# William-gregory/SeaIceExtentForecasting

Measured on AMD Instinct MI355X. Metric: GP fits/sec (n x n fp64, kernel+Cholesky+predict), higher is better.
Workload: dtype f64; 1 GPU; configs[2]: n=8192 d=8 fp64 RBF GPR, 40 retrospective years x hyper-parameter grid, one step = fits_per_step fits in lockstep; lockstep_group_asked=160, grid=smoke, parallelism=years sharded over 1 GPU(s), no data-path collective

## Files before the change

### include/sigp_debug.h

```cpp
#ifndef SIGP_DEBUG_H
#define SIGP_DEBUG_H
#include "sigp.h"
#ifdef __cplusplus
extern "C" {
#endif
int sigp_debug_diag_stamps(sigp_handle* h, const double* A128, double* out_us, int nout);
int sigp_debug_time_diag(sigp_handle* h, const double* A128, int skip, int reps, double* ms_avg, double* L_out, double* Linv_out);
int sigp_debug_time_kbuild(sigp_handle* h, int n, int d, int nb, int kernel_id, int flags, int reps, double* ms_avg);
int sigp_debug_mfma_peak(sigp_handle* h, int blocks, int iters, double* tflops, double seed);
int sigp_debug_time_syrk(sigp_handle* h, int rt, int K, int patch, int small, int reps, double* ms_avg, double* tflops, int dbg,
                         double* clock_ghz);
int sigp_debug_stream_concurrency(sigp_handle* h, int nstreams, int reps, int blocks, int iters, int use_slot_streams, double* ms_out);
int sigp_debug_cumask_probe(sigp_handle* h, const unsigned* mask8, int blocks, unsigned* out2);

int sigp_debug_run_gemm(sigp_handle* h, int dtype, int cfg, const void* A, int64_t lda, const void* B, int64_t ldb, void* C, int64_t ldc, int K, int r0, int r1,
                        int c0, int c1, int lower, int ktri, int batch, int64_t sA, int64_t sB, int64_t sC, int zcount, int64_t zA, int64_t zB, int64_t zC,
                        int zshift, int ride_bi1, int ride_rows, int64_t a_elems, int64_t b_elems, int64_t c_elems);
int sigp_debug_run_strip(sigp_handle* h, int dtype, void* M, int64_t ld, const void* Mt, int64_t ldm, int rb0, int nstrips, int J, int Wp, int members, int64_t sM,
                         int64_t sMt, int64_t m_elems, int64_t mt_elems);
int sigp_debug_run_link(sigp_handle* h, int dtype, void* M, int64_t ld, int c, const void* Linv, void* scratch, int rows_ride, int members, int64_t sM, int64_t sL,
                        int64_t sS, int64_t m_elems, int64_t linv_elems, int64_t scratch_elems);
int sigp_debug_run_refined_solve(sigp_handle* h, int trans, void* A, int64_t lda, int rows, const void* W, int64_t ldw, const void* L, int64_t ldl, int members,
                                 int64_t sA, int64_t sW, int64_t sL, int64_t a_elems, int64_t w_elems, int64_t l_elems);

int sigp_debug_run_rowdot(sigp_handle* h, int dtype, const void* Mx, int64_t ld, int nrows, int K, int kmode, const void* Zin, int64_t ldzin, void* Zout, int64_t ldzout,
                          int nrhs, int sub, const void* Zadd, int pm_pw, int j_off, int members, int64_t sM, int64_t sZi, int64_t sZo, int64_t m_elems,
                          int64_t zin_elems, int64_t zout_elems);
int sigp_debug_run_coldot(sigp_handle* h, int dtype, const void* Mx, int64_t ld, int ncols, int K, const void* Zin, int64_t ldzin, void* Zout, int64_t ldzout, int nrhs,
                          int64_t m_elems, int64_t zin_elems, int64_t zout_elems);
int sigp_debug_f32_solve(sigp_handle* h, int which, double* rhs, int64_t n, int nrhs);
int sigp_debug_f32_get_inverse(sigp_handle* h, int which, float* out);
int sigp_debug_run_hindcast_adjoint(sigp_handle* h, int64_t lead, int64_t min_train, int sigma_mode, int criterion, double* out, int64_t ldo);
int sigp_debug_run_hindcast_w(sigp_handle* h, int which, const double* U, const double* Cb, const double* z, const double* zbar, double* W, int n, int n_pad,
                              int64_t ld, int lead, int members, int64_t sC, int64_t sZ, int64_t c_elems, int64_t z_elems);
// ... 15 lines not shown
```

### seaiceextentforecasting_amd/csrc/gemm_mfma.hpp

```cpp
#pragma once
#include <hip/hip_runtime.h>

namespace sigp {

typedef double d4 __attribute__((ext_vector_type(4)));
typedef double d2 __attribute__((ext_vector_type(2)));
typedef float f4 __attribute__((ext_vector_type(4)));
typedef float f2 __attribute__((ext_vector_type(2)));

template <typename T> struct Num;
template <> struct Num<double> {
  typedef d4 acc_t;  typedef d2 v16_t;  typedef d2 v2_t;
  static constexpr int NE = 2;
  static constexpr int KT = 16;
  static constexpr int LDP = 18;
  __device__ static inline acc_t mfma(double a, double b, acc_t c) { return __builtin_amdgcn_mfma_f64_16x16x4f64(a, b, c, 0, 0, 0); }
  __device__ static inline int drow(int lq, int r) { return lq + 4 * r; }
  __device__ static inline int cswz(int R) { return (R & 1) << 3; }
};
template <> struct Num<float> {
  typedef f4 acc_t;  typedef f4 v16_t;  typedef f2 v2_t;
  static constexpr int NE = 4;
  static constexpr int KT = 32;
  static constexpr int LDP = 36;
  __device__ static inline acc_t mfma(float a, float b, acc_t c) { return __builtin_amdgcn_mfma_f32_16x16x4f32(a, b, c, 0, 0, 0); }
  __device__ static inline int drow(int lq, int r) { return 4 * lq + r; }
  __device__ static inline int cswz(int R) { return ((R >> 2) & 3) << 2; }
};

constexpr int KT = Num<double>::KT;

// ... 279 lines not shown
```

### seaiceextentforecasting_amd/csrc/sigp.hip

```cpp
#include <hip/hip_runtime.h>

#include <algorithm>
#include <cmath>
#include <cstdarg>
#include <cstdio>
#include <cstring>
#include <functional>
#include <limits>
#ifdef SIGP_DEBUG_TOOLS
#include <map>
#endif
#include <mutex>
#include <thread>
#include <chrono>
#include <string>
#include <type_traits>
#include <vector>

#include "../../include/sigp.h"
#include <dlfcn.h>
#include <rccl/rccl.h>
#include "gemm_mfma.hpp"
#include "kernels_misc.hpp"
#include "potrf_diag.hpp"
// ... 169 lines not shown
  bool built = false, factored = false, fitted = false;
  double sigma_f = 0, nlml = 0;
  KParams kp{};
  bool outer_set = false;
  int opt_outer = 8;
  int opt_lookahead = 1;
  int opt_small_tiles = 320;
  int opt_tiny_tiles = 256;
  int opt_pan_priority = 1;
  int opt_panel_ll = 0;
  int opt_panel_mode = 2;
  int opt_strip_min = 512;
  int opt_diag_tiles = 1;
  int opt_ride_tiles = 1;
  int opt_accurate = 0;
  int opt_strip_tri = 1;
  int opt_update_dbg = 0;
  int opt_c_dma = 0;
  int ncu = 256;
  int opt_ride_reps = 0;
  int opt_kbuild_mfma = 2;
  int opt_diag_prio = 1;
  int opt_schedule = 0;
  int opt_trsm128 = 256;
  int opt_n64_tiles = 0;
  int opt_wide_tiles = 0;
  int opt_syrk_v2 = 1;
  int opt_patch = 0;
  int opt_xcd_chunks = 0;
  int opt_first_on_panel = 1;
// ... 189 lines not shown
template <typename T, int TM, int TN, int WM, int WN, int MODE, bool BT>
int launch_gemm_cfg(sigp_handle* h, hipStream_t st, const GemmArgsT<T>& g) {
  const int nt = gemm_grid_size(g.r0, g.r1, g.c0, g.c1, g.lower, g.patch);
  if (nt <= 0) return SIGP_OK;
  auto kern = gemm_mfma_kernel<T, TM, TN, WM, WN, MODE, BT>;
  constexpr int lds = gemm_lds_bytes<T, TM, TN, BT>();
  static AttrOnce attr;
  HIPCHK(h, attr.set(h->device, (const void*)kern, lds));
  hipLaunchKernelGGL(kern, dim3(nt, std::max(1, g.batch), std::max(1, g.zcount)), dim3(256), lds, st, g);
  HIPCHK(h, hipGetLastError());
  return SIGP_OK;
}
template <int TM, int TN, int WM, int WN, int MODE, bool BT>
int launch_gemm_cfg(sigp_handle* h, hipStream_t st, const GemmArgs& g) { return launch_gemm_cfg<double, TM, TN, WM, WN, MODE, BT>(h, st, g); }

template <typename T, bool SET>
int launch_syrk128_t(sigp_handle* h, hipStream_t st, const GemmArgsT<T>& g, bool may_persist = false) {
  const int nt = gemm_grid_size(g.r0, g.r1, g.c0, g.c1, g.lower, g.patch);
  if (nt <= 0) return SIGP_OK;
  if (!sy_row_stride_ok(g.lda, sizeof(T)) || !sy_row_stride_ok(g.ldb, sizeof(T))) return fail(h, SIGP_BAD_ARG, "syrk128: operand row stride beyond the tile's 32-bit DMA offsets");
  static AttrOnce attr;
  HIPCHK(h, attr.set(h->device, (const void*)syrk128_kernel<T, SET>, SY_LDS_BYTES));
#ifdef SIGP_DEBUG_TOOLS
  if (g.dbg & (3 | 512)) {
    auto go = [&](auto abl) -> int {
      constexpr int A = decltype(abl)::value;
      static AttrOnce attr_a;
      HIPCHK(h, attr_a.set(h->device, (const void*)syrk128_kernel<T, SET, false, A>, SY_LDS_BYTES));
      hipLaunchKernelGGL((syrk128_kernel<T, SET, false, A>), dim3(nt, std::max(1, g.batch), std::max(1, g.zcount)), dim3(256), SY_LDS_BYTES, st, g);
      HIPCHK(h, hipGetLastError());
      return SIGP_OK;
    };
    switch ((g.dbg & 3) | ((g.dbg & 512) ? 4 : 0)) {
      case 1: return go(std::integral_constant<int, 1>{});
      case 2: return go(std::integral_constant<int, 2>{});
// ... 34 lines not shown
    hipLaunchKernelGGL((syrk128_kernel<T, SET, true>), dim3(h->opt_update_wgs, 1), dim3(256), SY_LDS_BYTES, st, gp);
    HIPCHK(h, hipGetLastError());
    return SIGP_OK;
  }
  if (may_persist && h->opt_xcd_chunks > 0 && g.lower && g.patch == 0 && g.r0 <= g.c0 && total >= 512) {
    GemmArgsT<T> gc = g;
    gc.patch = -h->opt_xcd_chunks; gc.ntile = nt;
    hipLaunchKernelGGL((syrk128_kernel<T, SET>), dim3((unsigned)round_up(total, 512), 1), dim3(256), SY_LDS_BYTES, st, gc);
    HIPCHK(h, hipGetLastError());
    return SIGP_OK;
  }
#else
  (void)may_persist;
#endif
  if constexpr (!SET) {
    if (h->opt_diag_tiles && g.lower && g.A == g.B && g.lda == g.ldb && g.sA == g.sB && g.zA == g.zB && g.r0 <= g.c0) {
      static AttrOnce attr_d;
      HIPCHK(h, attr_d.set(h->device, (const void*)syrk128_kernel<T, false, false, 0, true>, SY_LDS_BYTES));
      hipLaunchKernelGGL((syrk128_kernel<T, false, false, 0, true>), dim3(nt, std::max(1, g.batch), std::max(1, g.zcount)), dim3(256), SY_LDS_BYTES, st, g);
      HIPCHK(h, hipGetLastError());
      return SIGP_OK;
    }
  }
  hipLaunchKernelGGL((syrk128_kernel<T, SET>), dim3(nt, std::max(1, g.batch), std::max(1, g.zcount)), dim3(256), SY_LDS_BYTES, st, g);
  HIPCHK(h, hipGetLastError());
  return SIGP_OK;
}
int launch_syrk128(sigp_handle* h, hipStream_t st, const GemmArgs& g) { return launch_syrk128_t<double, false>(h, st, g); }

template <typename T>
int gemm_sub_auto(sigp_handle* h, hipStream_t st, GemmArgsT<T> g ) {
  const int nb = std::max(1, g.batch);
  const double nt1 = gemm_tile_count(g.r0, g.r1, g.c0, g.c1, g.lower);
  const int nt = (int)nt1 * nb;
// ... 325 lines not shown
    h->opt_cov_slices = (int)value; return SIGP_OK;
  }
  if (!strcmp(name, "cv_slices")) {
    if (value < 0 || value > 4096) return fail(h, SIGP_BAD_ARG, "cv_slices: 0 (auto) or 1 .. 4096 slices required (got %lld)", (long long)value);
    h->opt_cv_slices = (int)value; return SIGP_OK;
  }
  if (!strcmp(name, "loo_grad_tri")) { h->opt_loo_grad_tri = value != 0; return SIGP_OK; }
  if (!strcmp(name, "diag_tiles")) { h->opt_diag_tiles = value != 0; return SIGP_OK; }
  if (!strcmp(name, "ride_tiles")) { h->opt_ride_tiles = value != 0; return SIGP_OK; }
  if (!strcmp(name, "accurate_solve")) {
    if (h->dtype != SIGP_F64) return fail(h, SIGP_BAD_ARG, "accurate_solve: the fp64 engine's option (the fp32 engine refines against K~ itself)");
    if (value != 0 && value != 1) return fail(h, SIGP_BAD_ARG, "accurate_solve: 0 or 1 required (got %lld)", (long long)value);
    h->opt_accurate = (int)value; return SIGP_OK;
  }
  if (!strcmp(name, "strip_tri")) { h->opt_strip_tri = value != 0; return SIGP_OK; }
  if (!strcmp(name, "strip_min")) { if (value < 1) return SIGP_BAD_ARG; h->opt_strip_min = (int)value; return SIGP_OK; }
  if (!strcmp(name, "schedule")) { if (value < 0 || value > 1) return SIGP_BAD_ARG; h->opt_schedule = (int)value; return SIGP_OK; }
  if (!strcmp(name, "small_nt64")) { h->opt_small_nt64 = value != 0; return SIGP_OK; }
  if (!strcmp(name, "owner_only")) { h->opt_owner_only = value != 0; return SIGP_OK; }
  if (!strcmp(name, "dist_timeout_ms")) { if (value < 0) return SIGP_BAD_ARG; h->opt_dist_timeout_ms = (long)value; return SIGP_OK; }
  if (!strcmp(name, "dist_stats")) { h->opt_dist_stats = value != 0; return SIGP_OK; }
  if (!strcmp(name, "dist_panel_split")) { if (value < -1 || value > 1) return SIGP_BAD_ARG; h->opt_dist_split = (int)value; return SIGP_OK; }
  if (!strcmp(name, "dist_lookahead2d")) { h->opt_dist_la2d = value != 0; return SIGP_OK; }
  if (!strcmp(name, "dist_segment")) { if (value < 1 || value > 64) return SIGP_BAD_ARG; h->opt_dist_seg = (int)value; return SIGP_OK; }
  if (!strcmp(name, "panel_ll")) { if (value < 0 || value > 64) return SIGP_BAD_ARG; h->opt_panel_ll = (int)value; return SIGP_OK; }
  if (!strcmp(name, "trsm128_threshold")) { if (value < 0) return SIGP_BAD_ARG; h->opt_trsm128 = (int)value; return SIGP_OK; }
  if (!strcmp(name, "syrk_v2")) {
    if (!DBG_MASK) return fail(h, SIGP_BAD_ARG, "syrk_v2 is a measurement switch of libsigp_debug.so");
    h->opt_syrk_v2 = value ? 1 : 0; return SIGP_OK;
  }
// ... 937 lines not shown
```

### seaiceextentforecasting_amd/csrc/sigp_debug.inc

```
__global__ __launch_bounds__(256, 2) void mfma_peak_kernel(double* out, int iters, double seed) {
  sigp::d4 acc[16];
#pragma unroll
  for (int i = 0; i < 16; ++i) acc[i] = sigp::d4{0.0, 0.0, 0.0, 0.0};
  double a[8], b[8];
  unsigned long long x = 88172645463325252ull + threadIdx.x * 2654435761ull + blockIdx.x * 97ull;
#pragma unroll
  for (int i = 0; i < 8; ++i) {
    x ^= x << 13; x ^= x >> 7; x ^= x << 17;
    a[i] = seed < 0 ? (double)(long long)(x >> 11) * (1.0 / 9007199254740992.0) - 0.5 : seed + threadIdx.x * 1e-3;
    x ^= x << 13; x ^= x >> 7; x ^= x << 17;
    b[i] = seed < 0 ? (double)(long long)(x >> 11) * (1.0 / 9007199254740992.0) - 0.5 : seed - threadIdx.x * 1e-3;
  }
  for (int it = 0; it < iters; ++it) {
#pragma unroll
    for (int i = 0; i < 16; ++i) acc[i] = __builtin_amdgcn_mfma_f64_16x16x4f64(a[i & 7], b[(i + (i >> 3)) & 7], acc[i], 0, 0, 0);
  }
  double s = 0;
#pragma unroll
  for (int i = 0; i < 16; ++i) s += acc[i][0] + acc[i][1] + acc[i][2] + acc[i][3];
  out[blockIdx.x * 256 + threadIdx.x] = s;
}

__global__ void whereami_kernel(unsigned* out) {
  long long t0 = clock64();
// ... 451 lines not shown
                        int zshift, int ride_bi1, int ride_rows, int64_t a_elems, int64_t b_elems, int64_t c_elems) {
  if (dtype == SIGP_F32)
    return debug_run_gemm_t<float>(h, cfg, A, lda, B, ldb, C, ldc, K, r0, r1, c0, c1, lower, ktri, batch, sA, sB, sC, zcount, zA, zB, zC, zshift, ride_bi1, ride_rows,
                                   a_elems, b_elems, c_elems);
  if (dtype != SIGP_F64) return SIGP_BAD_ARG;
  return debug_run_gemm_t<double>(h, cfg, A, lda, B, ldb, C, ldc, K, r0, r1, c0, c1, lower, ktri, batch, sA, sB, sC, zcount, zA, zB, zC, zshift, ride_bi1, ride_rows,
                                  a_elems, b_elems, c_elems);
}

int sigp_debug_run_strip(sigp_handle* h, int dtype, void* M, int64_t ld, const void* Mt, int64_t ldm, int rb0, int nstrips, int J, int Wp, int members, int64_t sM,
                         int64_t sMt, int64_t m_elems, int64_t mt_elems) {
  if (dtype == SIGP_F32) return debug_run_strip_t<float>(h, M, ld, Mt, ldm, rb0, nstrips, J, Wp, members, sM, sMt, m_elems, mt_elems);
  if (dtype != SIGP_F64) return SIGP_BAD_ARG;
  return debug_run_strip_t<double>(h, M, ld, Mt, ldm, rb0, nstrips, J, Wp, members, sM, sMt, m_elems, mt_elems);
}

int sigp_debug_run_link(sigp_handle* h, int dtype, void* M, int64_t ld, int c, const void* Linv, void* scratch, int rows_ride, int members, int64_t sM, int64_t sL,
                        int64_t sS, int64_t m_elems, int64_t linv_elems, int64_t scratch_elems) {
  if (dtype == SIGP_F32) return debug_run_link_t<float>(h, M, ld, c, Linv, scratch, rows_ride, members, sM, sL, sS, m_elems, linv_elems, scratch_elems);
  if (dtype != SIGP_F64) return SIGP_BAD_ARG;
  return debug_run_link_t<double>(h, M, ld, c, Linv, scratch, rows_ride, members, sM, sL, sS, m_elems, linv_elems, scratch_elems);
}

int sigp_debug_run_refined_solve(sigp_handle* h, int trans, void* A, int64_t lda, int rows, const void* W, int64_t ldw, const void* L, int64_t ldl, int members,
                                 int64_t sA, int64_t sW, int64_t sL, int64_t a_elems, int64_t w_elems, int64_t l_elems) {
  constexpr long LIM = 1L << 20;
  if (!h || !A || !W || !L) return SIGP_BAD_ARG;
  if (h->dtype != SIGP_F64) return fail(h, SIGP_BAD_ARG, "debug_run_refined_solve: fp64 only");
  if ((trans != 0 && trans != 1) || rows < 1 || rows > LIM || members < 1 || members > 64) return fail(h, SIGP_BAD_ARG, "debug_run_refined_solve: trans / rows / members");
  if (lda < NB || ldw < NB || ldl < NB || lda > LIM || ldw > LIM || ldl > LIM || sA < 0 || sW < 0 || sL < 0 || std::max({sA, sW, sL}) > (1L << 40) || a_elems < 1 ||
// ... 345 lines not shown
```

### seaiceextentforecasting_amd/csrc/sigp_factor.inc

```

template <typename Real>
struct FactorView {
  Real* M; long ld, matStride;
  Real* dinv; long dinvStride;
  int nb;
  int* info;
  Real* lk;
  Real* at(long rblk, long cblk) const { return M + rblk * NB * ld + cblk * NB; }
  Real* dinv_at(long cblk) const { return dinv + cblk * NB * NB; }
};
template <typename Real>
FactorView<Real> member_view(Slot& s, Real* Mm, long ld, Real* dinvp) {
  return FactorView<Real>{Mm, ld, 0L, dinvp, 0L, 1, s.info, (Real*)s.lk};
}

struct PanelOpts {
  int ll = 0;
  bool leaf_pairs = false;
  int patch = 0;
  int ride_R = 0, ride_rows = 0;
};

template <typename Real>
int diag_block(sigp_handle* h, const FactorView<Real>& v, hipStream_t st, int c, const GemmArgsT<Real>* riding = nullptr, bool linked = false) {
// ... 17 lines not shown
  } else {
    HIPCHK(h, d_attr.set(h->device, (const void*)potrf_diag_kernel<Real>, diag_lds));
    hipLaunchKernelGGL(potrf_diag_kernel<Real>, dim3(nb), dim3(DIAG_THREADS), diag_lds, st, Ac, v.ld, v.dinv_at(c), v.info, c * NB, flags, v.matStride, v.dinvStride);
  }
  HIPCHK(h, hipGetLastError());
  return SIGP_OK;
}

template <typename Real>
int launch_column_solve(sigp_handle* h, hipStream_t st, GemmArgsT<Real> g, long rows, int nb) {
  if (rows <= 0) return SIGP_OK;
  g.batch = nb; g.K = NB; g.r0 = 0; g.c0 = 0; g.c1 = 1; g.lower = 0;
  ProfScope ps(h, st, SIGP_KC_TRSM, nb * 2.0 * rows * NB * NB * NB, nb * 2.0 * rows * NB * NB * 8);
  if (rows * nb >= h->opt_trsm128) {
    g.r1 = (int)rows;
    return launch_syrk128_t<Real, true>(h, st, g);
  }
  g.r1 = (int)rows * 4;
  return launch_gemm_cfg<Real, 32, 128, 1, 4, GEMM_SET, false>(h, st, g);
}
template <bool TRANS>
int launch_refined_solve(sigp_handle* h, hipStream_t st, const RefinedArgs& a, int nb) {
  if (a.rows <= 0 || nb <= 0) return SIGP_OK;
  static AttrOnce r_attr;
  ProfScope ps(h, st, SIGP_KC_TRSM, nb * 3.0 * 2.0 * a.rows * NB * NB, nb * (2.0 * a.rows * NB + 2.0 * NB * NB) * 8);
  HIPCHK(h, r_attr.set(h->device, (const void*)refined_solve_kernel<TRANS>, refined_lds_bytes()));
  hipLaunchKernelGGL(refined_solve_kernel<TRANS>, dim3((unsigned)((a.rows + RS_TM - 1) / RS_TM), (unsigned)nb), dim3(256), refined_lds_bytes(), st, a);
  HIPCHK(h, hipGetLastError());
  return SIGP_OK;
}
template <typename Real>
// ... 315 lines not shown
```

### seaiceextentforecasting_amd/csrc/syrk128.hpp

```cpp
#pragma once
#include <hip/hip_runtime.h>
#include <type_traits>

#include "gemm_mfma.hpp"

namespace sigp {

constexpr int SY_T = 128;
constexpr int SY_SLICE_BYTES = 128;
constexpr int SY_LDS_BYTES = 2 * 2 * SY_T * SY_SLICE_BYTES;
constexpr int SY_LDS_LONE_BYTES = 96 * 1024;

__host__ __device__ constexpr bool sy_row_stride_ok(long ld, int elem_bytes) { return ld > 0 && ld * elem_bytes < (1L << 25); }

typedef __attribute__((address_space(3))) void* lds_ptr_t;
typedef const __attribute__((address_space(1))) void* gbl_ptr_t;

template <typename T, bool SET, int ABL = 0, bool TRI = false, int WNC = 0, int DG = 0, int RD = 0>
__device__ __forceinline__ void syrk128_tile(const T* Ag, long lda, const T* Bg, long ldb, T* Cw,
                                             long ldc, int K, int dbg_in, T* As, T* Bs, bool stamp_in, unsigned long long& ph0, unsigned long long& ph1,
                                             int tid_in = -1) {
  static_assert(!TRI || (SET && sizeof(T) == 8), "TRI: fp64 strip solves only (C is not read)");
  static_assert(!DG || (!TRI && !SET), "DG: diagonal tiles of the trailing update");
  constexpr int IS = DG ? 32 : 16;
  constexpr int JS = (TRI || DG) ? 32 : 16;
  static_assert(!RD || (!TRI && !SET && !DG), "RD: ride-row tiles of the trailing update");
#define SY_NEED(i, j) (RD ? (RD == 1 && (i) == 0) : (DG == 0 || (DG == 1 ? (j) <= (i) : (j) < (i))))
  const int dbg = dbg_in & DBG_MASK;
  const bool stamp = stamp_in && DBG_MASK != 0;
  typedef Num<T> N_;
  typedef typename N_::acc_t acc_t;
  typedef typename N_::v16_t v16_t;
  constexpr int KTe = N_::KT, NE = N_::NE;
  const int tid = tid_in >= 0 ? tid_in : (int)threadIdx.x, lane = tid & 63, wave = __builtin_amdgcn_readfirstlane(tid >> 6);
  const int wm = wave >> 1, wn = TRI ? WNC : (wave & 1);
  const int lr = lane & 15, lq = lane >> 4;
  constexpr bool TRANSPOSED_ACC = sizeof(T) == 4;

  if (dbg & 8192) __builtin_amdgcn_s_setprio(3);
  if (dbg & 16384) __builtin_amdgcn_s_setprio(0);
  acc_t acc[4][4];
  if (SET || (dbg & 8)) {
#pragma unroll
    for (int i = 0; i < 4; ++i)
#pragma unroll
      for (int j = 0; j < 4; ++j)
#pragma unroll
        for (int r = 0; r < 4; ++r) acc[i][j][r] = (T)0;
  } else if (TRANSPOSED_ACC) {
#pragma unroll
    for (int i = 0; i < 4; ++i)
#pragma unroll
      for (int j = 0; j < 4; ++j) {
        if (!SY_NEED(i, j)) continue;
        const acc_t c = *(const acc_t*)(Cw + (long)(i * IS + lr) * ldc + j * JS + 4 * lq);
#pragma unroll
        for (int r = 0; r < 4; ++r) acc[i][j][r] = -c[r];
      }
  } else if (DG || !(dbg & 128)) {
#pragma unroll
    for (int i = 0; i < 4; ++i)
#pragma unroll
      for (int j = 0; j < 4; ++j)
        if (SY_NEED(i, j))
#pragma unroll
          for (int r = 0; r < 4; ++r) acc[i][j][r] = -Cw[(long)(i * IS + N_::drow(lq, r)) * ldc + j * JS + lr];
  } else {
    constexpr int CPR = SY_T / NE;
    constexpr int RPI = 64 / CPR;
    T* Cs = As;
    const T* Ctile = Cw - (long)(wm * 64) * ldc - wn * 64;
#pragma unroll
    for (int hh = 0; hh < 2; ++hh) {
      if (hh) __syncthreads();
#pragma unroll
      for (int q = 0; q < 16 / RPI; ++q) {
        const int R0 = wave * 16 + q * RPI;
        const int R = R0 + (lane / CPR), ch = lane % CPR;
        __builtin_amdgcn_global_load_lds((gbl_ptr_t)(Ctile + (long)(hh * 64 + R) * ldc + ((ch ^ N_::cswz(R)) * NE)),
                                         (lds_ptr_t)(Cs + R0 * SY_T), 16, 0, 0);
      }
      __syncthreads();
      if (wm == hh) {
#pragma unroll
        for (int i = 0; i < 4; ++i)
#pragma unroll
          for (int j = 0; j < 4; ++j)
#pragma unroll
            for (int r = 0; r < 4; ++r) {
              const int R = i * 16 + N_::drow(lq, r), col = wn * 64 + j * 16 + lr;
              acc[i][j][r] = -Cs[R * SY_T + (((col / NE) ^ N_::cswz(R)) * NE) + (col % NE)];
            }
      }
    }
    __syncthreads();
  }

  const int drow_ = wave * 8 + (lane >> 3);
  const int dks = ((lane & 7) ^ ((drow_ >> 1) & 7)) * NE;
  unsigned aoff[4], boff[4];
#pragma unroll
  for (int p = 0; p < 4; ++p) {
    aoff[p] = (unsigned)(((long)(drow_ + 32 * p) * lda + dks) * (long)sizeof(T));
    boff[p] = (unsigned)(((long)(drow_ + 32 * p) * ldb + dks) * (long)sizeof(T));
  }
#define SY_ISSUE(k0, buf)                                                                                     \
// ... 32 lines not shown
    constexpr int NP = NM < 8 ? NM : 8;
    const int buf = s & 1;
    const T* Ab = As + buf * SY_T * KTe + arow0;
    const T* Bb = Bs + buf * SY_T * KTe + brow0;
#pragma unroll
    for (int i = 0; i < 4; ++i) a1[i] = *(const v16_t*)(Ab + i * IS * KTe + fo1);
#pragma unroll
    for (int j = 0; j < 4; ++j) b1[j] = *(const v16_t*)(Bb + j * JS * KTe + fo1);
    if (!(ABL & 4))
#pragma unroll
    for (int e = 0; e < NE; ++e)
#pragma unroll
      for (int i = 0; i < 4; ++i)
#pragma unroll
        for (int j = JMIN; j < 4; ++j)
          if (SY_NEED(i, j)) acc[i][j] = TRANSPOSED_ACC ? N_::mfma(b0[j][e], a0[i][e], acc[i][j]) : N_::mfma(a0[i][e], b0[j][e], acc[i][j]);
#pragma unroll
    for (int q = 0; q < NP; ++q) {
      __builtin_amdgcn_sched_group_barrier(0x008, 1, 0);
      __builtin_amdgcn_sched_group_barrier(0x100, 1, 0);
    }
    if (NP < 8) __builtin_amdgcn_sched_group_barrier(0x100, 8 - NP, 0);
    if (NM > NP) __builtin_amdgcn_sched_group_barrier(0x008, NM - NP, 0);
    __builtin_amdgcn_sched_barrier(0);
    __syncthreads();
    __builtin_amdgcn_sched_barrier(0);
    if (decltype(with_dma)::value && !(ABL & 1)) SY_ISSUE((s + 2) * KTe, buf);
    if ((decltype(with_dma)::value || s + 1 < nst) && !(ABL & 2)) {
      const T* An = As + (buf ^ 1) * SY_T * KTe + arow0;
      const T* Bn = Bs + (buf ^ 1) * SY_T * KTe + brow0;
#pragma unroll
      for (int i = 0; i < 4; ++i) a0[i] = *(const v16_t*)(An + i * IS * KTe + fo0);
#pragma unroll
      for (int j = 0; j < 4; ++j) b0[j] = *(const v16_t*)(Bn + j * JS * KTe + fo0);
    }
    if (!(ABL & 4))
#pragma unroll
    for (int e = 0; e < NE; ++e)
#pragma unroll
      for (int i = 0; i < 4; ++i)
#pragma unroll
        for (int j = JMIN; j < 4; ++j)
          if (SY_NEED(i, j)) acc[i][j] = TRANSPOSED_ACC ? N_::mfma(b1[j][e], a1[i][e], acc[i][j]) : N_::mfma(a1[i][e], b1[j][e], acc[i][j]);
    if (decltype(with_dma)::value && NM >= 16) {
#pragma unroll
      for (int q = 0; q < 8; ++q) {
        __builtin_amdgcn_sched_group_barrier(0x010, 1, 1);
        __builtin_amdgcn_sched_group_barrier(0x008, 1, 1);
      }
#pragma unroll
      for (int q = 0; q < 8; ++q) {
        __builtin_amdgcn_sched_group_barrier(0x100, 1, 1);
        __builtin_amdgcn_sched_group_barrier(0x008, 1, 1);
      }
      if (NM > 16) __builtin_amdgcn_sched_group_barrier(0x008, NM - 16, 1);
    } else if (decltype(with_dma)::value && NM >= 8) {
#pragma unroll
      for (int q = 0; q < 8; ++q) {
// ... 19 lines not shown
      for (; s + 2 < nst; ++s) slice(s, std::true_type{}, J0_{});
      for (; s < nst; ++s) slice(s, std::false_type{}, J0_{});
    }
  }
#undef SY_ISSUE
  if (stamp) ph1 = __builtin_amdgcn_s_memtime();
  if (dbg & 8192) __builtin_amdgcn_s_setprio(3);
  if (dbg & 16384) __builtin_amdgcn_s_setprio(0);

  if (!(dbg & 16) || acc[0][0][0] == (T)12345.678) {
#pragma unroll
    for (int i = 0; i < 4; ++i)
#pragma unroll
      for (int j = 0; j < 4; ++j) {
        if (!SY_NEED(i, j)) continue;
        if (TRANSPOSED_ACC) {
          acc_t c;
#pragma unroll
          for (int r = 0; r < 4; ++r) c[r] = SET ? acc[i][j][r] : -acc[i][j][r];
          *(acc_t*)(Cw + (long)(i * IS + lr) * ldc + j * JS + 4 * lq) = c;
        } else {
#pragma unroll
          for (int r = 0; r < 4; ++r) Cw[(long)(i * IS + N_::drow(lq, r)) * ldc + j * JS + lr] = SET ? acc[i][j][r] : -acc[i][j][r];
        }
      }
  }
#undef SY_NEED
}

template <typename T, bool SET, bool PERSIST = false, int ABL = 0, bool DIAG_SKIP = false>
__global__ __launch_bounds__(256, 2) void syrk128_kernel(GemmArgsT<T> g) {
  static_assert(!DIAG_SKIP || (!SET && ABL == 0), "DIAG_SKIP: the product trailing update only");
  static_assert(!(DIAG_SKIP && PERSIST) || DBG_MASK != 0, "the persistent walk of the product instantiation: measured, not shipped (debug library only)");
  constexpr int KTe = Num<T>::KT;
  extern __shared__ __attribute__((aligned(16))) char smem_raw[];
  T* As = (T*)smem_raw;
  T* Bs = As + 2 * SY_T * KTe;
  const int tid = threadIdx.x, wave = __builtin_amdgcn_readfirstlane(tid >> 6);
  const int wm = wave >> 1, wn = wave & 1;
  unsigned long long* const stamp = DBG_MASK ? g.stamp : nullptr;
  const int total = PERSIST ? g.ntile * max(1, g.batch) : 1;
  for (int t = PERSIST ? (int)blockIdx.x : 0; t < total; t += PERSIST ? (int)gridDim.x : 1) {
    int bi, bj;
    long bz;
    if (PERSIST) {
      bz = t / g.ntile;
      if (!gemm_tile_coords(g, t - (int)bz * g.ntile, bi, bj)) continue;
    } else if (g.patch < 0) {
      if (!gemm_tile_coords_chunked(g, blockIdx.x, bi, bj, bz)) return;
    } else {
      bz = blockIdx.y;
      if (!gemm_tile_coords(g, blockIdx.x, bi, bj)) return;
    }
    const long zz = (long)blockIdx.z;
    const T* Ag = g.A + bz * g.sA + zz * g.zA + (long)bi * SY_T * g.lda;
    const T* Bg = g.B + bz * g.sB + zz * g.zB + (long)bj * SY_T * g.ldb;
    int K = g.K;
    if (g.ktri == 1) { const int ks = bi * SY_T; Ag += ks; Bg += ks; K -= ks; }
    T* Cw = g.C + bz * g.sC + zz * g.zC + ((long)bi * SY_T + wm * 64) * g.ldc + (long)bj * SY_T + wn * 64;
    const bool diag = DIAG_SKIP && g.lower && bi == bj && g.A == g.B && g.sA == g.sB && g.zA == g.zB && g.lda == g.ldb;
    unsigned long long st_c0 = 0, st_r0 = 0;
    if (stamp) { st_c0 = __builtin_amdgcn_s_memtime(); st_r0 = __builtin_amdgcn_s_memrealtime(); }
    unsigned long long ph0 = 0, ph1 = 0;
    int tid_t = tid;
    if (PERSIST || DIAG_SKIP) asm volatile("" : "+v"(tid_t));
    const bool ride = DIAG_SKIP && g.ride_bi1 > 0 && bi == g.ride_bi1 - 1;
    if (DIAG_SKIP && ride) {
      if (wm == 0) syrk128_tile<T, SET, ABL, false, 0, 0, DIAG_SKIP ? 1 : 0>(Ag, g.lda, Bg, g.ldb, Cw, g.ldc, K, g.dbg, As, Bs, stamp != nullptr, ph0, ph1, tid_t);
      else syrk128_tile<T, SET, ABL, false, 0, 0, DIAG_SKIP ? 2 : 0>(Ag, g.lda, Bg, g.ldb, Cw, g.ldc, K, g.dbg, As, Bs, stamp != nullptr, ph0, ph1, tid_t);
    } else if (DIAG_SKIP && diag) {
      T* Cd = g.C + bz * g.sC + zz * g.zC + ((long)bi * SY_T + wm * 16) * g.ldc + (long)bj * SY_T + wn * 16;
      if (wave == 1) syrk128_tile<T, SET, ABL, false, 0, DIAG_SKIP ? 2 : 0>(Ag, g.lda, Bg, g.ldb, Cd, g.ldc, K, g.dbg, As, Bs, stamp != nullptr, ph0, ph1, tid_t);
      else syrk128_tile<T, SET, ABL, false, 0, DIAG_SKIP ? 1 : 0>(Ag, g.lda, Bg, g.ldb, Cd, g.ldc, K, g.dbg, As, Bs, stamp != nullptr, ph0, ph1, tid_t);
    } else {
      syrk128_tile<T, SET, ABL>(Ag, g.lda, Bg, g.ldb, Cw, g.ldc, K, g.dbg, As, Bs, stamp != nullptr, ph0, ph1, tid_t);
    }
    const size_t st_i = PERSIST ? (size_t)t : (size_t)blockIdx.y * gridDim.x + blockIdx.x, st_n = PERSIST ? (size_t)total : (size_t)gridDim.x * gridDim.y;
    if (stamp && (g.dbg & 256)) {
      __builtin_amdgcn_s_waitcnt(0);
      if (tid == 0) {
        unsigned long long* o = stamp + 2 * st_n + 3 * st_i;
        o[0] = ph0 - st_c0; o[1] = ph1 - ph0; o[2] = __builtin_amdgcn_s_memtime() - ph1;
      }
    }
    if (stamp && tid == 0) {
      stamp[2 * st_i] = __builtin_amdgcn_s_memtime() - st_c0;
      stamp[2 * st_i + 1] = ((__builtin_amdgcn_s_memrealtime() - st_r0) << 8) | (__builtin_amdgcn_s_getreg((20 << 0) | (0 << 6) | (31 << 11)) & 0xf);
    }
    if (stamp && (g.dbg & 4096) && (tid & 63) == 0) {
      unsigned long long* o = stamp + 5 * st_n + 8 * st_i;
// ... 55 lines not shown
```

Baseline: 344.1 fits/s.

## Use MFMA negate modifier, scalar-base C addressing, and triangular solve tile in syrk128

The fp64 trailing-update path now uses the MFMA negate-A modifier, so C -= A B^T no longer needs C negated on load and store. It also adds a scalar-base addressing form for loading and storing the C tile, which cuts per-element 64-bit VGPR address arithmetic. The triangular-solve (SET) launch gets a BTRI instantiation that uses the triangular tile variant with narrower column offsets, skipping work in the triangular B operand. All three are on by default behind new options, at the cost of more template instantiations and a stricter ldc stride check.

```diff
diff --git a/include/sigp_debug.h b/include/sigp_debug.h
--- a/include/sigp_debug.h
+++ b/include/sigp_debug.h
@@ -18,6 +18,7 @@
                         int zshift, int ride_bi1, int ride_rows, int64_t a_elems, int64_t b_elems, int64_t c_elems);
 int sigp_debug_run_strip(sigp_handle* h, int dtype, void* M, int64_t ld, const void* Mt, int64_t ldm, int rb0, int nstrips, int J, int Wp, int members, int64_t sM,
                          int64_t sMt, int64_t m_elems, int64_t mt_elems);
+int sigp_debug_syrk128_strides(sigp_handle* h, int dtype, int64_t lda, int64_t ldb, int64_t ldc);
 int sigp_debug_run_link(sigp_handle* h, int dtype, void* M, int64_t ld, int c, const void* Linv, void* scratch, int rows_ride, int members, int64_t sM, int64_t sL,
                         int64_t sS, int64_t m_elems, int64_t linv_elems, int64_t scratch_elems);
 int sigp_debug_run_refined_solve(sigp_handle* h, int trans, void* A, int64_t lda, int rows, const void* W, int64_t ldw, const void* L, int64_t ldl, int members,
diff --git a/seaiceextentforecasting_amd/csrc/gemm_mfma.hpp b/seaiceextentforecasting_amd/csrc/gemm_mfma.hpp
--- a/seaiceextentforecasting_amd/csrc/gemm_mfma.hpp
+++ b/seaiceextentforecasting_amd/csrc/gemm_mfma.hpp
@@ -15,6 +15,7 @@
   static constexpr int KT = 16;
   static constexpr int LDP = 18;
   __device__ static inline acc_t mfma(double a, double b, acc_t c) { return __builtin_amdgcn_mfma_f64_16x16x4f64(a, b, c, 0, 0, 0); }
+  __device__ static inline acc_t mfma_nega(double a, double b, acc_t c) { return __builtin_amdgcn_mfma_f64_16x16x4f64(a, b, c, 0, 0, 1); }
   __device__ static inline int drow(int lq, int r) { return lq + 4 * r; }
   __device__ static inline int cswz(int R) { return (R & 1) << 3; }
 };
diff --git a/seaiceextentforecasting_amd/csrc/sigp.hip b/seaiceextentforecasting_amd/csrc/sigp.hip
--- a/seaiceextentforecasting_amd/csrc/sigp.hip
+++ b/seaiceextentforecasting_amd/csrc/sigp.hip
@@ -207,6 +207,9 @@
   int opt_diag_tiles = 1;
   int opt_ride_tiles = 1;
   int opt_accurate = 0;
+  int opt_mfma_neg = 1;
+  int opt_c_sbase = 1;
+  int opt_solve_tri = 1;
   int opt_strip_tri = 1;
   int opt_update_dbg = 0;
   int opt_c_dma = 0;
@@ -426,11 +429,17 @@
 template <int TM, int TN, int WM, int WN, int MODE, bool BT>
 int launch_gemm_cfg(sigp_handle* h, hipStream_t st, const GemmArgs& g) { return launch_gemm_cfg<double, TM, TN, WM, WN, MODE, BT>(h, st, g); }
 
+template <typename T>
+int syrk128_check_strides(sigp_handle* h, long lda, long ldb, long ldc) {
+  if (!sy_row_stride_ok(lda, sizeof(T)) || !sy_row_stride_ok(ldb, sizeof(T)) || !sy_row_stride_ok(ldc, sizeof(T)))
+    return fail(h, SIGP_BAD_ARG, "syrk128: row stride beyond the tile's 32-bit offsets");
+  return SIGP_OK;
+}
 template <typename T, bool SET>
-int launch_syrk128_t(sigp_handle* h, hipStream_t st, const GemmArgsT<T>& g, bool may_persist = false) {
+int launch_syrk128_t(sigp_handle* h, hipStream_t st, const GemmArgsT<T>& g, bool may_persist = false, bool b_tri = false) {
   const int nt = gemm_grid_size(g.r0, g.r1, g.c0, g.c1, g.lower, g.patch);
   if (nt <= 0) return SIGP_OK;
-  if (!sy_row_stride_ok(g.lda, sizeof(T)) || !sy_row_stride_ok(g.ldb, sizeof(T))) return fail(h, SIGP_BAD_ARG, "syrk128: operand row stride beyond the tile's 32-bit DMA offsets");
+  if (const int rcs = syrk128_check_strides<T>(h, g.lda, g.ldb, g.ldc)) return rcs;
   static AttrOnce attr;
   HIPCHK(h, attr.set(h->device, (const void*)syrk128_kernel<T, SET>, SY_LDS_BYTES));
 #ifdef SIGP_DEBUG_TOOLS
@@ -495,10 +504,29 @@
   (void)may_persist;
 #endif
   if constexpr (!SET) {
-    if (h->opt_diag_tiles && g.lower && g.A == g.B && g.lda == g.ldb && g.sA == g.sB && g.zA == g.zB && g.r0 <= g.c0) {
-      static AttrOnce attr_d;
-      HIPCHK(h, attr_d.set(h->device, (const void*)syrk128_kernel<T, false, false, 0, true>, SY_LDS_BYTES));
-      hipLaunchKernelGGL((syrk128_kernel<T, false, false, 0, true>), dim3(nt, std::max(1, g.batch), std::max(1, g.zcount)), dim3(256), SY_LDS_BYTES, st, g);
+    const bool sym = h->opt_diag_tiles && g.lower && g.A == g.B && g.lda == g.ldb && g.sA == g.sB && g.zA == g.zB && g.r0 <= g.c0;
+    const bool nega = sizeof(T) == 8 && h->opt_mfma_neg;
+    const bool csb = sizeof(T) == 8 && h->opt_c_sbase;
+    auto go = [&](auto skip, auto form) -> int {
+      constexpr bool SK = decltype(skip)::value, NG = sizeof(T) == 8 && (decltype(form)::value & 1), SB = sizeof(T) == 8 && (decltype(form)::value & 2);
+      static AttrOnce attr_f;
+      HIPCHK(h, attr_f.set(h->device, (const void*)syrk128_kernel<T, false, false, 0, SK, NG, false, SB>, SY_LDS_BYTES));
+      hipLaunchKernelGGL((syrk128_kernel<T, false, false, 0, SK, NG, false, SB>), dim3(nt, std::max(1, g.batch), std::max(1, g.zcount)), dim3(256), SY_LDS_BYTES, st, g);
+      HIPCHK(h, hipGetLastError());
+      return SIGP_OK;
+    };
+    typedef std::integral_constant<int, 1> F1; typedef std::integral_constant<int, 2> F2; typedef std::integral_constant<int, 3> F3;
+    switch ((nega ? 1 : 0) | (csb ? 2 : 0)) {
+      case 3: return sym ? go(std::true_type{}, F3{}) : go(std::false_type{}, F3{});
+      case 2: return sym ? go(std::true_type{}, F2{}) : go(std::false_type{}, F2{});
+      case 1: return sym ? go(std::true_type{}, F1{}) : go(std::false_type{}, F1{});
+      default: if (sym) return go(std::true_type{}, std::integral_constant<int, 0>{});
+    }
+  } else if constexpr (sizeof(T) == 8) {
+    if (b_tri && h->opt_solve_tri && g.K == SY_T && g.ktri == 0) {
+      static AttrOnce attr_t;
+      HIPCHK(h, attr_t.set(h->device, (const void*)syrk128_kernel<T, true, false, 0, false, false, true>, SY_LDS_BYTES));
+      hipLaunchKernelGGL((syrk128_kernel<T, true, false, 0, false, false, true>), dim3(nt, std::max(1, g.batch), std::max(1, g.zcount)), dim3(256), SY_LDS_BYTES, st, g);
       HIPCHK(h, hipGetLastError());
       return SIGP_OK;
     }
@@ -854,6 +882,9 @@
     h->opt_accurate = (int)value; return SIGP_OK;
   }
   if (!strcmp(name, "strip_tri")) { h->opt_strip_tri = value != 0; return SIGP_OK; }
+  if (!strcmp(name, "mfma_neg")) { h->opt_mfma_neg = value != 0; return SIGP_OK; }
+  if (!strcmp(name, "c_sbase")) { h->opt_c_sbase = value != 0; return SIGP_OK; }
+  if (!strcmp(name, "solve_tri")) { h->opt_solve_tri = value != 0; return SIGP_OK; }
   if (!strcmp(name, "strip_min")) { if (value < 1) return SIGP_BAD_ARG; h->opt_strip_min = (int)value; return SIGP_OK; }
   if (!strcmp(name, "schedule")) { if (value < 0 || value > 1) return SIGP_BAD_ARG; h->opt_schedule = (int)value; return SIGP_OK; }
   if (!strcmp(name, "small_nt64")) { h->opt_small_nt64 = value != 0; return SIGP_OK; }
diff --git a/seaiceextentforecasting_amd/csrc/sigp_debug.inc b/seaiceextentforecasting_amd/csrc/sigp_debug.inc
--- a/seaiceextentforecasting_amd/csrc/sigp_debug.inc
+++ b/seaiceextentforecasting_amd/csrc/sigp_debug.inc
@@ -489,6 +489,10 @@
   if (dtype != SIGP_F64) return SIGP_BAD_ARG;
   return debug_run_strip_t<double>(h, M, ld, Mt, ldm, rb0, nstrips, J, Wp, members, sM, sMt, m_elems, mt_elems);
 }
+int sigp_debug_syrk128_strides(sigp_handle* h, int dtype, int64_t lda, int64_t ldb, int64_t ldc) {
+  if (!h) return SIGP_BAD_ARG;
+  return dtype == SIGP_F32 ? syrk128_check_strides<float>(h, lda, ldb, ldc) : syrk128_check_strides<double>(h, lda, ldb, ldc);
+}
 
 int sigp_debug_run_link(sigp_handle* h, int dtype, void* M, int64_t ld, int c, const void* Linv, void* scratch, int rows_ride, int members, int64_t sM, int64_t sL,
                         int64_t sS, int64_t m_elems, int64_t linv_elems, int64_t scratch_elems) {
diff --git a/seaiceextentforecasting_amd/csrc/sigp_factor.inc b/seaiceextentforecasting_amd/csrc/sigp_factor.inc
--- a/seaiceextentforecasting_amd/csrc/sigp_factor.inc
+++ b/seaiceextentforecasting_amd/csrc/sigp_factor.inc
@@ -55,7 +55,7 @@
   ProfScope ps(h, st, SIGP_KC_TRSM, nb * 2.0 * rows * NB * NB * NB, nb * 2.0 * rows * NB * NB * 8);
   if (rows * nb >= h->opt_trsm128) {
     g.r1 = (int)rows;
-    return launch_syrk128_t<Real, true>(h, st, g);
+    return launch_syrk128_t<Real, true>(h, st, g, false, true);
   }
   g.r1 = (int)rows * 4;
   return launch_gemm_cfg<Real, 32, 128, 1, 4, GEMM_SET, false>(h, st, g);
diff --git a/seaiceextentforecasting_amd/csrc/syrk128.hpp b/seaiceextentforecasting_amd/csrc/syrk128.hpp
--- a/seaiceextentforecasting_amd/csrc/syrk128.hpp
+++ b/seaiceextentforecasting_amd/csrc/syrk128.hpp
@@ -16,7 +16,13 @@
 typedef __attribute__((address_space(3))) void* lds_ptr_t;
 typedef const __attribute__((address_space(1))) void* gbl_ptr_t;
 
-template <typename T, bool SET, int ABL = 0, bool TRI = false, int WNC = 0, int DG = 0, int RD = 0>
+template <typename T, bool NEGA>
+__device__ __forceinline__ typename Num<T>::acc_t sy_mfma(T a, T b, typename Num<T>::acc_t c) {
+  if constexpr (NEGA) return Num<T>::mfma_nega(a, b, c);
+  else return Num<T>::mfma(a, b, c);
+}
+
+template <typename T, bool SET, int ABL = 0, bool TRI = false, int WNC = 0, int DG = 0, int RD = 0, bool NEGA = false, bool CSB = false>
 __device__ __forceinline__ void syrk128_tile(const T* Ag, long lda, const T* Bg, long ldb, T* Cw,
                                              long ldc, int K, int dbg_in, T* As, T* Bs, bool stamp_in, unsigned long long& ph0, unsigned long long& ph1,
                                              int tid_in = -1) {
@@ -25,6 +31,10 @@
   constexpr int IS = DG ? 32 : 16;
   constexpr int JS = (TRI || DG) ? 32 : 16;
   static_assert(!RD || (!TRI && !SET && !DG), "RD: ride-row tiles of the trailing update");
+  static_assert(!NEGA || (!SET && sizeof(T) == 8), "NEGA: the fp64 MFMA's negate-A modifier, C -= A B^T");
+  static_assert(!CSB || (!SET && sizeof(T) == 8), "CSB: scalar-base C addressing of the fp64 update tile");
+  constexpr bool FLIP = !SET && !NEGA;
+#define SY_MFMA(a, b, c) sy_mfma<T, NEGA>(a, b, c)
 #define SY_NEED(i, j) (RD ? (RD == 1 && (i) == 0) : (DG == 0 || (DG == 1 ? (j) <= (i) : (j) < (i))))
   const int dbg = dbg_in & DBG_MASK;
   const bool stamp = stamp_in && DBG_MASK != 0;
@@ -55,7 +65,24 @@
         if (!SY_NEED(i, j)) continue;
         const acc_t c = *(const acc_t*)(Cw + (long)(i * IS + lr) * ldc + j * JS + 4 * lq);
 #pragma unroll
-        for (int r = 0; r < 4; ++r) acc[i][j][r] = -c[r];
+        for (int r = 0; r < 4; ++r) acc[i][j][r] = FLIP ? -c[r] : c[r];
+      }
+  } else if (CSB && (DG || !(dbg & 128))) {
+    unsigned coff = (unsigned)(((long)lq * ldc + lr) * (long)sizeof(T));
+#pragma unroll
+    for (int i = 0; i < 4; ++i)
+#pragma unroll
+      for (int r = 0; r < 4; ++r) {
+        if (!SY_NEED(i, 0) && !SY_NEED(i, 3)) continue;
+        unsigned long cb = (unsigned long)(Cw + (long)(i * IS + 4 * r) * ldc);
+        asm("" : "+s"(cb));
+        asm("" : "+v"(coff));
+#pragma unroll
+        for (int j = 0; j < 4; ++j)
+          if (SY_NEED(i, j)) {
+            const T c = *(const __attribute__((address_space(1))) T*)((const __attribute__((address_space(1))) char*)cb + coff + j * JS * (int)sizeof(T));
+            acc[i][j][r] = FLIP ? -c : c;
+          }
       }
   } else if (DG || !(dbg & 128)) {
 #pragma unroll
@@ -64,7 +91,10 @@
       for (int j = 0; j < 4; ++j)
         if (SY_NEED(i, j))
 #pragma unroll
-          for (int r = 0; r < 4; ++r) acc[i][j][r] = -Cw[(long)(i * IS + N_::drow(lq, r)) * ldc + j * JS + lr];
+          for (int r = 0; r < 4; ++r) {
+            const T c = Cw[(long)(i * IS + N_::drow(lq, r)) * ldc + j * JS + lr];
+            acc[i][j][r] = FLIP ? -c : c;
+          }
   } else {
     constexpr int CPR = SY_T / NE;
     constexpr int RPI = 64 / CPR;
@@ -89,7 +119,8 @@
 #pragma unroll
             for (int r = 0; r < 4; ++r) {
               const int R = i * 16 + N_::drow(lq, r), col = wn * 64 + j * 16 + lr;
-              acc[i][j][r] = -Cs[R * SY_T + (((col / NE) ^ N_::cswz(R)) * NE) + (col % NE)];
+              const T c = Cs[R * SY_T + (((col / NE) ^ N_::cswz(R)) * NE) + (col % NE)];
+              acc[i][j][r] = FLIP ? -c : c;
             }
       }
     }
@@ -152,7 +183,7 @@
       for (int i = 0; i < 4; ++i)
 #pragma unroll
         for (int j = JMIN; j < 4; ++j)
-          if (SY_NEED(i, j)) acc[i][j] = TRANSPOSED_ACC ? N_::mfma(b0[j][e], a0[i][e], acc[i][j]) : N_::mfma(a0[i][e], b0[j][e], acc[i][j]);
+          if (SY_NEED(i, j)) acc[i][j] = TRANSPOSED_ACC ? N_::mfma(b0[j][e], a0[i][e], acc[i][j]) : SY_MFMA(a0[i][e], b0[j][e], acc[i][j]);
 #pragma unroll
     for (int q = 0; q < NP; ++q) {
       __builtin_amdgcn_sched_group_barrier(0x008, 1, 0);
@@ -179,7 +210,7 @@
       for (int i = 0; i < 4; ++i)
 #pragma unroll
         for (int j = JMIN; j < 4; ++j)
-          if (SY_NEED(i, j)) acc[i][j] = TRANSPOSED_ACC ? N_::mfma(b1[j][e], a1[i][e], acc[i][j]) : N_::mfma(a1[i][e], b1[j][e], acc[i][j]);
+          if (SY_NEED(i, j)) acc[i][j] = TRANSPOSED_ACC ? N_::mfma(b1[j][e], a1[i][e], acc[i][j]) : SY_MFMA(a1[i][e], b1[j][e], acc[i][j]);
     if (decltype(with_dma)::value && NM >= 16) {
 #pragma unroll
       for (int q = 0; q < 8; ++q) {
@@ -229,23 +260,41 @@
 #pragma unroll
       for (int j = 0; j < 4; ++j) {
         if (!SY_NEED(i, j)) continue;
+        if (CSB) continue;
         if (TRANSPOSED_ACC) {
           acc_t c;
 #pragma unroll
-          for (int r = 0; r < 4; ++r) c[r] = SET ? acc[i][j][r] : -acc[i][j][r];
+          for (int r = 0; r < 4; ++r) c[r] = FLIP ? -acc[i][j][r] : acc[i][j][r];
           *(acc_t*)(Cw + (long)(i * IS + lr) * ldc + j * JS + 4 * lq) = c;
         } else {
 #pragma unroll
-          for (int r = 0; r < 4; ++r) Cw[(long)(i * IS + N_::drow(lq, r)) * ldc + j * JS + lr] = SET ? acc[i][j][r] : -acc[i][j][r];
+          for (int r = 0; r < 4; ++r) Cw[(long)(i * IS + N_::drow(lq, r)) * ldc + j * JS + lr] = FLIP ? -acc[i][j][r] : acc[i][j][r];
         }
       }
+    if (CSB) {
+      unsigned coff = (unsigned)(((long)lq * ldc + lr) * (long)sizeof(T));
+#pragma unroll
+      for (int i = 0; i < 4; ++i)
+#pragma unroll
+        for (int r = 0; r < 4; ++r) {
+          if (!SY_NEED(i, 0) && !SY_NEED(i, 3)) continue;
+          unsigned long cb = (unsigned long)(Cw + (long)(i * IS + 4 * r) * ldc);
+          asm("" : "+s"(cb));
+          asm("" : "+v"(coff));
+#pragma unroll
+          for (int j = 0; j < 4; ++j)
+            if (SY_NEED(i, j)) *(__attribute__((address_space(1))) T*)((__attribute__((address_space(1))) char*)cb + coff + j * JS * (int)sizeof(T)) = FLIP ? -acc[i][j][r] : acc[i][j][r];
+        }
+    }
   }
 #undef SY_NEED
-}
-
-template <typename T, bool SET, bool PERSIST = false, int ABL = 0, bool DIAG_SKIP = false>
+#undef SY_MFMA
+}
+
+template <typename T, bool SET, bool PERSIST = false, int ABL = 0, bool DIAG_SKIP = false, bool NEGA = false, bool BTRI = false, bool CSB = false>
 __global__ __launch_bounds__(256, 2) void syrk128_kernel(GemmArgsT<T> g) {
   static_assert(!DIAG_SKIP || (!SET && ABL == 0), "DIAG_SKIP: the product trailing update only");
+  static_assert(!BTRI || (SET && !PERSIST && ABL == 0 && !DIAG_SKIP && sizeof(T) == 8), "BTRI: the fp64 column solve only");
   static_assert(!(DIAG_SKIP && PERSIST) || DBG_MASK != 0, "the persistent walk of the product instantiation: measured, not shipped (debug library only)");
   constexpr int KTe = Num<T>::KT;
   extern __shared__ __attribute__((aligned(16))) char smem_raw[];
@@ -272,23 +321,26 @@
     const T* Bg = g.B + bz * g.sB + zz * g.zB + (long)bj * SY_T * g.ldb;
     int K = g.K;
     if (g.ktri == 1) { const int ks = bi * SY_T; Ag += ks; Bg += ks; K -= ks; }
-    T* Cw = g.C + bz * g.sC + zz * g.zC + ((long)bi * SY_T + wm * 64) * g.ldc + (long)bj * SY_T + wn * 64;
+    T* Cw = g.C + bz * g.sC + zz * g.zC + ((long)bi * SY_T + wm * 64) * g.ldc + (long)bj * SY_T + wn * (BTRI ? 16 : 64);
     const bool diag = DIAG_SKIP && g.lower && bi == bj && g.A == g.B && g.sA == g.sB && g.zA == g.zB && g.lda == g.ldb;
     unsigned long long st_c0 = 0, st_r0 = 0;
     if (stamp) { st_c0 = __builtin_amdgcn_s_memtime(); st_r0 = __builtin_amdgcn_s_memrealtime(); }
     unsigned long long ph0 = 0, ph1 = 0;
     int tid_t = tid;
-    if (PERSIST || DIAG_SKIP) asm volatile("" : "+v"(tid_t));
+    if (PERSIST || DIAG_SKIP || BTRI) asm volatile("" : "+v"(tid_t));
     const bool ride = DIAG_SKIP && g.ride_bi1 > 0 && bi == g.ride_bi1 - 1;
-    if (DIAG_SKIP && ride) {
-      if (wm == 0) syrk128_tile<T, SET, ABL, false, 0, 0, DIAG_SKIP ? 1 : 0>(Ag, g.lda, Bg, g.ldb, Cw, g.ldc, K, g.dbg, As, Bs, stamp != nullptr, ph0, ph1, tid_t);
-      else syrk128_tile<T, SET, ABL, false, 0, 0, DIAG_SKIP ? 2 : 0>(Ag, g.lda, Bg, g.ldb, Cw, g.ldc, K, g.dbg, As, Bs, stamp != nullptr, ph0, ph1, tid_t);
+    if constexpr (BTRI) {
+      if (wn == 0) syrk128_tile<T, true, 0, true, 0>(Ag, g.lda, Bg, g.ldb, Cw, g.ldc, K, g.dbg, As, Bs, stamp != nullptr, ph0, ph1, tid_t);
+      else syrk128_tile<T, true, 0, true, 1>(Ag, g.lda, Bg, g.ldb, Cw, g.ldc, K, g.dbg, As, Bs, stamp != nullptr, ph0, ph1, tid_t);
+    } else if (DIAG_SKIP && ride) {
+      if (wm == 0) syrk128_tile<T, SET, ABL, false, 0, 0, DIAG_SKIP ? 1 : 0, NEGA, CSB>(Ag, g.lda, Bg, g.ldb, Cw, g.ldc, K, g.dbg, As, Bs, stamp != nullptr, ph0, ph1, tid_t);
+      else syrk128_tile<T, SET, ABL, false, 0, 0, DIAG_SKIP ? 2 : 0, NEGA, CSB>(Ag, g.lda, Bg, g.ldb, Cw, g.ldc, K, g.dbg, As, Bs, stamp != nullptr, ph0, ph1, tid_t);
     } else if (DIAG_SKIP && diag) {
       T* Cd = g.C + bz * g.sC + zz * g.zC + ((long)bi * SY_T + wm * 16) * g.ldc + (long)bj * SY_T + wn * 16;
-      if (wave == 1) syrk128_tile<T, SET, ABL, false, 0, DIAG_SKIP ? 2 : 0>(Ag, g.lda, Bg, g.ldb, Cd, g.ldc, K, g.dbg, As, Bs, stamp != nullptr, ph0, ph1, tid_t);
-      else syrk128_tile<T, SET, ABL, false, 0, DIAG_SKIP ? 1 : 0>(Ag, g.lda, Bg, g.ldb, Cd, g.ldc, K, g.dbg, As, Bs, stamp != nullptr, ph0, ph1, tid_t);
+      if (wave == 1) syrk128_tile<T, SET, ABL, false, 0, DIAG_SKIP ? 2 : 0, 0, NEGA, CSB>(Ag, g.lda, Bg, g.ldb, Cd, g.ldc, K, g.dbg, As, Bs, stamp != nullptr, ph0, ph1, tid_t);
+      else syrk128_tile<T, SET, ABL, false, 0, DIAG_SKIP ? 1 : 0, 0, NEGA, CSB>(Ag, g.lda, Bg, g.ldb, Cd, g.ldc, K, g.dbg, As, Bs, stamp != nullptr, ph0, ph1, tid_t);
     } else {
-      syrk128_tile<T, SET, ABL>(Ag, g.lda, Bg, g.ldb, Cw, g.ldc, K, g.dbg, As, Bs, stamp != nullptr, ph0, ph1, tid_t);
+      syrk128_tile<T, SET, ABL, false, 0, 0, 0, NEGA, CSB>(Ag, g.lda, Bg, g.ldb, Cw, g.ldc, K, g.dbg, As, Bs, stamp != nullptr, ph0, ph1, tid_t);
     }
     const size_t st_i = PERSIST ? (size_t)t : (size_t)blockIdx.y * gridDim.x + blockIdx.x, st_n = PERSIST ? (size_t)total : (size_t)gridDim.x * gridDim.y;
     if (stamp && (g.dbg & 256)) {
```

Result: no change. 345.4 fits/s (median of 6 runs) (+0.4%).
